# trifectatechfoundation/zlib-rs

Hardware: NVIDIA H100
Metric: deflate_level6_raw_input_throughput_silesia_small_tar (higher is better)
Workload: dtype u8

## Files before the change

__graft_entry__.py:

```python
import os
import subprocess
import sys

ROOT = os.path.dirname(os.path.abspath(__file__))
if ROOT not in sys.path:
    sys.path.insert(0, ROOT)
sys.path.insert(0, os.path.join(ROOT, "tests"))


def build():
    subprocess.check_call(["make", "-C", os.path.join(ROOT, "zlib_rs_b200", "csrc"), "-j8"])
    subprocess.check_call(["make", "-C", os.path.join(ROOT, "oracle")])
    subprocess.check_call(["make", "-C", os.path.join(ROOT, "oracle"), "ref"])
    subprocess.check_call(["make", "-C", os.path.join(ROOT, "tests", "hostmodel")])
    subprocess.check_call(["make", "-C", os.path.join(ROOT, "tests", "shardmodel")])
    subprocess.check_call(["make", "-C", os.path.join(ROOT, "tests", "membermodel")])
    subprocess.check_call(["make", "-C", os.path.join(ROOT, "tests", "bgzfmodel")])
    subprocess.check_call(["make", "-C", os.path.join(ROOT, "tests", "batchmodel")])
    subprocess.check_call(["make", "-C", os.path.join(ROOT, "tests", "batchdictmodel")])
    subprocess.check_call(["make", "-C", os.path.join(ROOT, "tests", "batchdictsmodel")])
    subprocess.check_call(["make", "-C", os.path.join(ROOT, "tests", "batchparammodel")])
    subprocess.check_call(["make", "-C", os.path.join(ROOT, "tests", "indexmodel")])
    subprocess.check_call(["make", "-C", os.path.join(ROOT, "tests", "writerindexmodel")])
    subprocess.check_call(["make", "-C", os.path.join(ROOT, "tests", "flushmodel")])
    subprocess.check_call(["make", "-C", os.path.join(ROOT, "tests", "bgzfindexmodel")])
    subprocess.check_call(["make", "-C", os.path.join(ROOT, "tests", "c_client")])
    import zlib_rs_b200
    zlib_rs_b200.lib()


def smoke():
    import zlib
    import zlib_rs_b200 as Z
    import oracle_lib as O
    from corpus import synthetic_mix
    d = synthetic_mix(300000, seed=1)
    out = Z.compress2(d, 6)
    assert out == O.compress(d, 6)[1], "GPU deflate differs from the oracle"
    assert zlib.decompress(out) == d
    assert Z.uncompress(out, len(d)) == d
    assert Z.crc32(d) == O.crc32(d) and Z.adler32(d) == O.adler32(d)
    print("smoke ok: %d -> %d bytes, bit-exact vs oracle" % (len(d), len(out)))


if __name__ == "__main__":
    build()
    if len(sys.argv) > 1 and sys.argv[1] == "smoke":
        smoke()
```

zlib_rs_b200/csrc/zb_core.h:

```cpp
#pragma once
#include <stdint.h>

#if defined(__CUDACC__)
#define ZB_HD __host__ __device__ __forceinline__
#define ZB_HDN __host__ __device__
#else
#define ZB_HD inline
#define ZB_HDN
#endif

namespace zb {

constexpr uint32_t kWSize = 32768;
constexpr uint32_t kMaxDist = kWSize - 262;
constexpr uint32_t kMinLookahead = 262;
constexpr uint32_t kT0 = 2 * kWSize - 262;
constexpr uint32_t kMaxMatch = 258;
constexpr uint32_t kLitBufsize = 16384;
constexpr uint32_t kBlockSyms = kLitBufsize - 1;
constexpr uint32_t kTailZone = 1024;
constexpr uint32_t kMSafe = 640;
constexpr uint32_t kPad = 1024;

ZB_HD uint32_t zlib_level_flags(uint32_t level, bool plain_strategy)
// ... 19 lines not shown
    }
}
ZB_HD void stream_trailer(uint8_t *t, uint32_t wrap, uint32_t check, uint32_t isize)
{
    if (wrap == 1) {
        for (int i = 0; i < 4; i++) t[i] = (uint8_t)(check >> (24 - 8 * i));
    } else if (wrap == 2) {
        for (int i = 0; i < 4; i++) { t[i] = (uint8_t)(check >> (8 * i)); t[4 + i] = (uint8_t)(isize >> (8 * i)); }
    }
}
constexpr uint32_t kStoredMax = 65535;
ZB_HD uint64_t stored_blocks(uint64_t n) { return n == 0 ? 1 : (n + kStoredMax - 1) / kStoredMax; }
ZB_HD uint64_t stored_payload(uint64_t n) { return n + 5 * stored_blocks(n); }
ZB_HD void stored_header(uint8_t *p, uint32_t len, bool last)
{
    p[0] = last ? 1 : 0;
    p[1] = (uint8_t)len;
    p[2] = (uint8_t)(len >> 8);
    p[3] = (uint8_t)~len;
    p[4] = (uint8_t)(~len >> 8);
}

struct LevelParams {
    uint32_t good, lazy, nice, chain;
    uint32_t early_exit;
};
ZB_HD LevelParams level_params(int level)
{
    switch (level) {
    case 3: return {4, 6, 16, 6, 1};
    case 4: return {4, 12, 32, 24, 1};
    case 5: return {8, 16, 32, 32, 0};
    default: return {8, 16, 128, 128, 0};
    }
}

ZB_HD uint32_t hash_u32(uint32_t v) { return (v * 2654435761u) >> 16; }

struct FullWin {
    ZB_HD uint32_t wsize() const { return kWSize; }
    ZB_HD uint32_t maxdist() const { return kMaxDist; }
    ZB_HD uint32_t t0() const { return kT0; }
};
struct DynWin {
    uint32_t w;
    ZB_HD uint32_t wsize() const { return w; }
    ZB_HD uint32_t maxdist() const { return w - kMinLookahead; }
    ZB_HD uint32_t t0() const { return 2 * w - kMinLookahead; }
};
template <class WN>
ZB_HD uint32_t wbase_w(const WN &wn, uint32_t p) { return p <= wn.t0() ? 0u : wn.wsize() * (1u + (p - wn.t0() - 1u) / wn.wsize()); }

ZB_HD uint32_t wbase(uint32_t p) { return p <= kT0 ? 0u : kWSize * (1u + (p - kT0 - 1u) / kWSize); }


template <class A>
ZB_HD uint32_t common_prefix(const A &a, uint32_t x, uint32_t c, uint32_t maxlen)
{
    uint32_t n = 0;
    while (n < maxlen && a.byte(x + n) == a.byte(c + n)) n++;
    return n;
}

struct Match {
    uint32_t len;
    uint32_t start;
};

template <class A, class WN = FullWin>
ZB_HD Match lm_walk(const A &a, uint32_t x, uint32_t cap, const LevelParams &lp, const WN wn = WN())
{
    Match r{0, 0};
    uint32_t best = 2;
    uint32_t chain = lp.chain;
    uint32_t cur = x;
    bool first = true;
    for (;;) {
        uint32_t d = a.link(cur);
        if (d == 0) break;
        cur -= d;
        uint32_t dist = x - cur;
        if (dist > (first ? wn.maxdist() : wn.maxdist() - 1)) break;
        if (cur == 0) break;
        if (!a.inserted(cur)) continue;
        first = false;
        uint32_t len = 0;
        bool pass;
        if (best < 8) {
            uint32_t c8 = common_prefix(a, x, cur, 8);
            if (c8 == 8) { pass = true; }
            else if (c8 > best) { pass = true; len = c8; }
            else pass = false;
        } else {
            uint32_t off = best - 7;
            pass = common_prefix(a, x + off, cur + off, 8) == 8 && common_prefix(a, x, cur, 8) == 8;
        }
        if (pass) {
            if (len == 0) len = 2 + common_prefix(a, x + 2, cur + 2, 256);
            if (len > best) {
                r.start = cur;
                if (len >= cap) { r.len = cap; return r; }
                best = len;
                r.len = len;
                if (best >= lp.nice) return r;
            } else if (lp.early_exit) {
                break;
// ... 226 lines not shown
```

zlib_rs_b200/csrc/zb_engine.cu:

```cuda
#include <cuda_runtime.h>
#include <stdio.h>
#include <stdlib.h>
#include <string.h>
#include <algorithm>
#include <new>
#include "../../include/zb_engine.h"
#include "zb_kernels.cuh"
#include "zb_engine_internal.h"

namespace zb {

constexpr uint32_t kSlowSub9 = 24576;
constexpr uint32_t kTailTiles = 2;
constexpr uint32_t kTailSub = 512;

thread_local char g_err[256] = "";

static void set_err(const char *what, cudaError_t e)
{
    snprintf(g_err, sizeof g_err, "%s: %s", what, cudaGetErrorString(e));
}

#define CK(call)                                                  \
    do {                                                          \
        cudaError_t e_ = (call);                                  \
        if (e_ != cudaSuccess) { set_err(#call, e_); return ZB_E_CUDA; } \
    } while (0)

__global__ void k_match(JobBufs);
__global__ void k_skip(JobBufs);
__global__ void k_nxt(JobBufs);
__global__ void k_path_tiles(JobBufs);
__global__ void k_path_chain(JobBufs, uint32_t, uint32_t);
__global__ void k_path_groups(JobBufs, uint32_t, uint32_t, uint4 *, uint32_t *);
__global__ void k_path_chain2(JobBufs, uint32_t, uint32_t, const uint4 *, uint32_t *, uint32_t *);
__global__ void k_path_mark(JobBufs, const uint32_t *, const uint32_t *);
__global__ void k_iter_lists(JobBufs, uint32_t *, uint32_t *, uint32_t);
__global__ void k_emit(JobBufs);
__global__ void k_holes(JobBufs, uint32_t);
__global__ void k_holes_cmp(JobBufs, uint32_t, uint32_t);
__global__ void k_tail(JobBufs);
__global__ void k_block_hist(JobBufs, uint32_t *);
__global__ void k_build_blocks(JobBufs, const uint32_t *);
__global__ void k_scan_blocks(JobBufs);
__global__ void k_encode(JobBufs);
__global__ void k_finish(JobBufs, const uint32_t *);
__global__ void k_literal_syms(JobBufs);
__global__ void k_stored(JobBufs);
__global__ void k_links2_std(JobBufs, uint32_t);
__global__ void k_links2_roll(JobBufs, uint32_t);
__global__ void k_links_fix_std(JobBufs);
__global__ void k_links_fix_roll(JobBufs);
__global__ void k_slow(JobBufs);
__global__ void k_rle(JobBufs);
__global__ void k_emit_slow(JobBufs);
__global__ void k_tail_slow(JobBufs);
__global__ void k_serial_low(JobBufs);
__global__ void k_links_dict_ghost(JobBufs, uint32_t *);
__global__ void k_links_dict_ghost_apply(JobBufs, const uint32_t *);
__global__ void k_bgzf_setup(BgzfJob, uint64_t);
__global__ void k_serial_low_members(JobBufs, BgzfJob);
__global__ void k_bgzf_medium(JobBufs, BgzfJob);
__global__ void k_bgzf_slow_steps(JobBufs, BgzfJob);
__global__ void k_bgzf_slow_walk(JobBufs, BgzfJob);
__global__ void k_bgzf_rle_steps(JobBufs, BgzfJob);
__global__ void k_bgzf_literals(JobBufs, BgzfJob);
__global__ void k_bgzf_hist(JobBufs, BgzfJob, uint32_t *);
__global__ void k_bgzf_build(JobBufs, BgzfJob, const uint32_t *);
__global__ void k_bgzf_size(JobBufs, BgzfJob);
__global__ void k_bgzf_scan(JobBufs, BgzfJob);
__global__ void k_bgzf_encode(JobBufs, BgzfJob);
__global__ void k_bgzf_frame(JobBufs, BgzfJob);
__global__ void k_batch_stage(const uint8_t *, const uint64_t *, const uint8_t *, const uint64_t *, BgzfJob, uint8_t *, uint64_t);
__global__ void k_batch_dict_ghost(JobBufs, BgzfJob);
__global__ void k_flush_blocks(JobBufs, BgzfJob);
__global__ void k_deflate_points(JobBufs, BgzfJob, IdxWriteJob);

constexpr uint32_t kMatchSmemBytes = (kWSize + kMatchSub + 512) + (kWSize + kMatchSub) * 2 + ((kWSize + kMatchSub) / 32 + 1) * 4 * 4 + 8192;
constexpr uint32_t kPathSmemBytes = kPathTile * 4 * 3;
constexpr uint32_t kLinks2SmemBytes = 65536 * 2 + kLinkTile * 2 + kLinkTile + 64 + 2048;
constexpr uint32_t kSkipSmemBytes = 2 * kWSize * 2 + 2 * (2 * kWSize / 32) * 4 + 8192 + 64;
constexpr uint32_t kSlowSubMax = 24576;
constexpr uint32_t kSlowSmemBytes = (kWSize + kSlowSubMax + kSlowAhead) * 3;
constexpr uint32_t kChainSmemBytes = kChainChunkTiles * kPathHead * 8;
constexpr uint32_t kChain2MaxSmem = 200 * 1024;
constexpr uint32_t kSerialSmemBytes = (65536 + kWSize) * 2 + 35824 + 16;
constexpr uint32_t kSerialSmemQuick = 65536 * 2 + 65536 + 16;

int Engine::init(int dev)
{
    int n = 0;
    cudaError_t e = cudaGetDeviceCount(&n);
    if (e != cudaSuccess || n == 0) {
        snprintf(g_err, sizeof g_err, "no CUDA device (%s)", e == cudaSuccess ? "count 0" : cudaGetErrorString(e));
        return ZB_E_NODEVICE;
    }
    if (dev < 0 || dev >= n) { snprintf(g_err, sizeof g_err, "device %d out of range", dev); return ZB_E_PARAM; }
    device = dev;
    CK(cudaSetDevice(dev));
    CK(cudaStreamCreateWithFlags(&st, cudaStreamNonBlocking));
    CK(cudaStreamCreateWithFlags(&st2, cudaStreamNonBlocking));
    CK(cudaEventCreateWithFlags(&evf, cudaEventDisableTiming));
    CK(cudaEventCreateWithFlags(&evt, cudaEventDisableTiming));
    for (int i = 0; i < kUpChunks; i++) CK(cudaEventCreateWithFlags(&evc[i], cudaEventDisableTiming));
    CK(cudaEventCreateWithFlags(&evk, cudaEventDisableTiming));
    CK(cudaEventCreate(&ev0));
    CK(cudaEventCreate(&ev1));
    CK(upload_tables());
    CK(cudaFuncSetAttribute(k_match, cudaFuncAttributeMaxDynamicSharedMemorySize, kMatchSmemBytes));
    CK(cudaFuncSetAttribute(k_skip, cudaFuncAttributeMaxDynamicSharedMemorySize, kSkipSmemBytes));
    CK(cudaFuncSetAttribute(k_links2_std, cudaFuncAttributeMaxDynamicSharedMemorySize, kLinks2SmemBytes));
    CK(cudaFuncSetAttribute(k_links2_roll, cudaFuncAttributeMaxDynamicSharedMemorySize, kLinks2SmemBytes));
    CK(cudaFuncSetAttribute(k_slow, cudaFuncAttributeMaxDynamicSharedMemorySize, kSlowSmemBytes));
    CK(cudaFuncSetAttribute(k_path_tiles, cudaFuncAttributeMaxDynamicSharedMemorySize, kPathSmemBytes));
    CK(cudaFuncSetAttribute(k_path_mark, cudaFuncAttributeMaxDynamicSharedMemorySize, kPathSmemBytes));
    CK(cudaFuncSetAttribute(k_path_chain, cudaFuncAttributeMaxDynamicSharedMemorySize, kChainSmemBytes));
    CK(cudaFuncSetAttribute(k_path_groups, cudaFuncAttributeMaxDynamicSharedMemorySize, kChain2MaxSmem));
    CK(cudaFuncSetAttribute(k_path_chain2, cudaFuncAttributeMaxDynamicSharedMemorySize, kChain2MaxSmem));
    CK(cudaFuncSetAttribute(k_serial_low, cudaFuncAttributeMaxDynamicSharedMemorySize, kSerialSmemBytes));
    CK(cudaFuncSetAttribute(k_serial_low_members, cudaFuncAttributeMaxDynamicSharedMemorySize, kSerialSmemBytes));
    CK(cudaMallocHost(&h_info, sizeof(JobInfo)));
    CK(cudaMalloc(&d_info, sizeof(JobInfo)));
    CK(cudaMalloc(&d_check, 16));
    { int rc_ = inflate_init(); if (rc_ != ZB_OK) return rc_; }
    return ZB_OK;
}

Engine::~Engine()
{
    if (device < 0) return;
    cudaSetDevice(device);
    for (auto &b : bufs) if (b.p) cudaFree(b.p);
    if (h_stage) cudaFreeHost(h_stage);
    if (h_info) cudaFreeHost(h_info);
    if (d_info) cudaFree(d_info);
    if (d_check) cudaFree(d_check);
    if (ev0) cudaEventDestroy(ev0);
    if (ev1) cudaEventDestroy(ev1);
    if (evf) cudaEventDestroy(evf);
    if (evt) cudaEventDestroy(evt);
    for (int i = 0; i < kUpChunks; i++) if (evc[i]) cudaEventDestroy(evc[i]);
    if (evk) cudaEventDestroy(evk);
    if (st2) cudaStreamDestroy(st2);
    if (st) cudaStreamDestroy(st);
}

void Engine::pbegin()
{
    if (!profile) return;
    if (!pev0) { cudaEventCreate(&pev0); cudaEventCreate(&pev1); }
    cudaEventRecord(pev0, st);
}

void Engine::pend(int phase, uint32_t nlaunch)
{
    if (!profile) return;
    cudaEventRecord(pev1, st);
    cudaEventSynchronize(pev1);
    float ms = 0;
    cudaEventElapsedTime(&ms, pev0, pev1);
    phase_ms[phase] += ms;
    phase_launches[phase] += nlaunch;
}
// ... 58 lines not shown
    uint32_t wrap;
    if (window_bits < 0) { if (window_bits < -15 || window_bits > -8) return ZB_E_PARAM; wrap = 0; }
    else if (window_bits > 15) { if (window_bits < 24 || window_bits > 31) return ZB_E_PARAM; wrap = 2; }
    else { if (window_bits < 8) return ZB_E_PARAM; wrap = 1; }
    const int wb = window_bits < 0 ? -window_bits : window_bits > 15 ? window_bits - 16 : window_bits;
    CK(cudaSetDevice(device));
    const uint32_t N = (uint32_t)n;
    launches = 0;

    JobBufs jb;
    memset(&jb, 0, sizeof jb);
    int rc;
    void *p;
    const size_t npad = (size_t)N + kPad;
    const uint32_t nwords = (N >> 5) + 2;
    const uint32_t nmt = N / kMatchTile + 1, npt = N / kPathTile + 1;
    const bool low_parallel = (flags & ZB_FLAG_LOW_PARALLEL) != 0 || dstart != 0;
    const bool serial_low = (level == 1 || level == 2) && strategy != 2 && strategy != 3 && !low_parallel;
    const uint32_t block_syms = (serial_low && level == 1) ? kBlockSyms : (1u << (mem_level + 6)) - 1u;
    const uint32_t max_blocks = N / block_syms + 2;
    const size_t out_cap = (deflate_bound(n) + 15) & ~(size_t)15;
    if ((rc = stage((size_t)nmt + 64 + ((size_t)N / 512 + 2 + npt + nmt + 8) * 4 + 64)) != ZB_OK) return rc;
    uint8_t *h_dirty = static_cast<uint8_t *>(h_stage);
    uint32_t *h_lists = reinterpret_cast<uint32_t *>(static_cast<uint8_t *>(h_stage) + (((size_t)nmt + 64 + 15) & ~(size_t)15));
#define RES(slot, bytes, field, type)                                   \
    if ((rc = reserve(slot, bytes, &p)) != ZB_OK) return rc;            \
    jb.field = static_cast<type>(p);
    uint8_t *d_in;
    if ((rc = reserve(S_IN, npad + 16, &p)) != ZB_OK) return rc;
    d_in = static_cast<uint8_t *>(p);
    jb.in = d_in;
    jb.N = N;
    jb.start = (uint32_t)dstart;
    jb.nmt = nmt;
    jb.tail_start = N > 2 * kTailZone ? N - kTailZone : 0;
    jb.block_syms = block_syms;
    jb.serial_mode = serial_low ? (uint32_t)level : 0u;
    RES(S_L, npad * 2, L, uint16_t *)
    RES(S_SK, npad * 2, SK, uint16_t *)
    RES(S_HOLES, (size_t)nwords * 4, holes, uint32_t *)
    RES(S_HOLESN, (size_t)nwords * 4, holes_new, uint32_t *)
    RES(S_M, npad * 4, M, uint32_t *)
    RES(S_NXT, ((size_t)N + 16) * 4, nxt, uint32_t *)
    RES(S_PEXIT, ((size_t)N + 16) * 4, pexit, uint32_t *)
    RES(S_PCNT, ((size_t)N + 16) * 4, pcnt, uint32_t *)
    RES(S_SYMIDX, ((size_t)N + 16) * 4, symidx, uint32_t *)
    RES(S_PHEAD, (size_t)npt * kPathHead * 8, phead, uint2 *)
    RES(S_TENTRY, (size_t)npt * 4, tile_entry, uint32_t *)
    RES(S_TSYMB, (size_t)npt * 4, tile_symbase, uint32_t *)
    RES(S_MARKN, (size_t)npt + 16, mark_needed, uint8_t *)
    const uint32_t nlists = npt * (kPathTile / kPathSub);
    RES(S_LLIST, (size_t)nlists * kLongPerSub * 4, long_list, uint32_t *)
    RES(S_LCNT, (size_t)nlists * 4, long_cnt, uint32_t *)
    RES(S_TDIRTY, (size_t)nmt + 16, tile_dirty, uint8_t *)
    RES(S_SYMS, ((size_t)N + 64) * sizeof(Sym), syms, Sym *)
    RES(S_SYMB, 40000 * 4, sym_base, uint32_t *)
    RES(S_BMAP, (size_t)nmt * 8192, bucket_map, uint32_t *)
    RES(S_LR, npad * 2, Lr, uint16_t *)
    RES(S_KEYS, npad * 2, keys, uint16_t *)
    RES(S_LLAST, (size_t)nmt * 65536 * 2, link_last, uint16_t *)
    RES(S_CSTATE, (size_t)(npt + 1) * 16, chain_state, uint4 *)
    uint32_t chainG = 16;
    while ((uint64_t)chainG * chainG < npt) chainG += 8;
    const uint32_t chain_groups = (npt + chainG - 1) / chainG;
    const uint32_t chain2_smem = chainG * kPathHead * 8 + chain_groups * kPathHead * 16 + chainG * 8;
    const bool chain2 = chain2_smem <= kChain2MaxSmem;
    if ((rc = reserve(S_GFN, (size_t)chain_groups * kPathHead * 16 + ((size_t)npt + 4) * 4, &p)) != ZB_OK) return rc;
    uint4 *d_gfn = static_cast<uint4 *>(p);
    uint32_t *d_mark_cnt = reinterpret_cast<uint32_t *>(d_gfn + (size_t)chain_groups * kPathHead);
    uint32_t *d_mark_list = d_mark_cnt + 4;
    auto launch_chain = [&](uint32_t first_tile) {
        if (chain2) {
            k_path_groups<<<chain_groups, 1024, chainG * kPathHead * 8, st>>>(jb, npt, chainG, d_gfn, d_mark_cnt);
            k_path_chain2<<<chain_groups, 1024, chain2_smem, st>>>(jb, npt, chainG, d_gfn, d_mark_list, d_mark_cnt);
            launches++;
        } else k_path_chain<<<1, 1024, kChainSmemBytes, st>>>(jb, npt, first_tile);
    };
    auto launch_mark = [&](uint32_t grid) {
        if (chain2) k_path_mark<<<grid < npt ? grid : npt, 1024, kPathSmemBytes, st>>>(jb, d_mark_list, d_mark_cnt);
        else k_path_mark<<<npt, 1024, kPathSmemBytes, st>>>(jb, nullptr, nullptr);
    };
    uint32_t *d_lists;
    const uint32_t max_list = N / 512 + 2;
    if ((rc = reserve(S_LISTS, ((size_t)max_list + npt + nmt + 8) * 4, &p)) != ZB_OK) return rc;
    d_lists = static_cast<uint32_t *>(p);
    RES(S_HDIFF, (size_t)nwords * 8, hdiff, uint32_t *)
    jb.hdiff_words = nwords;
    RES(S_HCOARSE, (size_t)(N >> 10) + 16, hcoarse, uint8_t *)
    RES(S_MCHG, (((size_t)N >> 8) + 16) * 4 + 64, mchg, uint8_t *)
    RES(S_BLOCKS, (size_t)max_blocks * sizeof(BlockDesc), blocks, BlockDesc *)
    RES(S_BBASE, (size_t)max_blocks * 4, block_base, uint32_t *)
    uint32_t *d_freq;
    if ((rc = reserve(S_FREQ, (size_t)max_blocks * 320 * 4, &p)) != ZB_OK) return rc;
    d_freq = static_cast<uint32_t *>(p);
    uint8_t *d_out;
    if (dst_dev && dst_cap >= out_cap) d_out = static_cast<uint8_t *>(dst);
    else { if ((rc = reserve(S_OUT, out_cap + 16, &p)) != ZB_OK) return rc; d_out = static_cast<uint8_t *>(p); }
    jb.out = d_out;
    jb.out_cap = out_cap;
    void *d_ck;
    const size_t ck_bytes = ((size_t)N / 16384 + 16) * 8;
    if ((rc = reserve(S_CK, ck_bytes, &d_ck)) != ZB_OK) return rc;
#undef RES
    jb.info = d_info;
    jb.level = (uint32_t)level;
    jb.strategy_fixed = strategy == 4;
    const bool lf_zero = strategy >= 2;
// ... 71 lines not shown
        pend(9, 0);
    }
    CK(cudaMemsetAsync(d_info, 0, sizeof(JobInfo), st));
    CK(cudaMemsetAsync(d_out, 0, out_cap, st));
    if (jb.prime_bits) {
        h_prime = (uint8_t)((flags >> 16) & ((1u << jb.prime_bits) - 1u));
        CK(cudaMemcpyAsync(d_out, &h_prime, 1, cudaMemcpyHostToDevice, st));
    }
    cudaStream_t st_ck = chunked_upload ? st2 : st;
    pbegin();
    if (wrap == 1 || (wrap == 0 && (flags & ZB_FLAG_CHECK_ADLER))) { CK(launch_adler32(d_in + dstart, n_in, 1, d_ck, ck_bytes, d_check, st_ck)); launches += 2; }
    else if (wrap == 2 || (wrap == 0 && (flags & ZB_FLAG_CHECK_CRC))) { CK(launch_crc32(d_in + dstart, n_in, 0, d_ck, ck_bytes, d_check, st_ck)); launches += 2; }
    else CK(cudaMemsetAsync(d_check, 0, 4, st_ck));
    if (chunked_upload) CK(cudaEventRecord(evk, st2));
    pend(8, 2);

    auto links_tiles = [&](bool roll) {
        uint32_t t_done = 0;
        for (uint32_t k = 0; k < (chunked_upload ? up_chunks : 1u); k++) {
            uint32_t t_hi = nmt;
            if (chunked_upload) {
                cudaStreamWaitEvent(st, evc[k], 0);
                if (k + 1 < up_chunks) t_hi = up_len[k] >= 64 ? (uint32_t)((up_len[k] - 64) / kLinkTile) : 0;
            }
            if (t_hi <= t_done) continue;
            if (roll) k_links2_roll<<<t_hi - t_done, 1024, kLinks2SmemBytes, st>>>(jb, t_done);
            else k_links2_std<<<t_hi - t_done, 1024, kLinks2SmemBytes, st>>>(jb, t_done);
            if (k) launches++;
            t_done = t_hi;
        }
        if (chunked_upload) cudaStreamWaitEvent(st, evk, 0);
    };
    uint32_t iters = 0;
    if (level == 0) {
        const uint32_t nb = n_in == 0 ? 1 : (uint32_t)((n_in + 65534) / 65535);
        k_stored<<<nb, 256, 0, st>>>(jb);
        launches++;
        k_finish<<<1, 32, 0, st>>>(jb, d_check);
        launches++;
    } else {
        if (jb.huffman_only) {
            k_literal_syms<<<(uint32_t)(n_in / 256 + 1), 256, 0, st>>>(jb);
            launches++;
        } else if (jb.serial_mode) {
            iters = 1;
            pbegin();
            k_serial_low<<<1, 32, jb.serial_mode == 2 ? kSerialSmemBytes : kSerialSmemQuick, st>>>(jb);
            launches++;
            pend(1, 1);
        } else {
            CK(cudaMemsetAsync(jb.holes, 0, (size_t)nwords * 4, st));
            CK(cudaMemsetAsync(jb.holes_new, 0, (size_t)nwords * 4, st));
            CK(cudaMemsetAsync(jb.tile_dirty, 1, nmt, st));
            CK(cudaMemsetAsync(jb.tile_entry, 0xee, (size_t)npt * 4, st));
            CK(cudaMemsetAsync(jb.M + N, 0, (size_t)kPad * 4, st));
            CK(cudaMemsetAsync(jb.L + N, 0, (size_t)kPad * 2, st));
            pbegin();
            if (jb.slow_mode == 2) {
            } else if (jb.slow_mode && jb.sp.slow) {
                links_tiles(true);
                k_links_fix_roll<<<N / 256 + 1, 256, 0, st>>>(jb);
                launches += 2;
            } else {
                links_tiles(false);
                k_links_fix_std<<<N / 256 + 1, 256, 0, st>>>(jb);
                launches += 2;
                if (dstart >= 3 && n_in) {
                    uint32_t *d_first = reinterpret_cast<uint32_t *>(d_check) + 2;
                    CK(cudaMemsetAsync(d_first, 0xff, 4, st));
                    k_links_dict_ghost<<<(kMaxDist + 255) / 256, 256, 0, st>>>(jb, d_first);
                    k_links_dict_ghost_apply<<<1, 32, 0, st>>>(jb, d_first);
                    launches += 2;
                }
            }
            if (!jb.slow_mode) CK(cudaMemcpyAsync(jb.Lr, jb.L, npad * 2, cudaMemcpyDeviceToDevice, st));
            pend(0, 1);
            if (jb.slow_mode) {
                if (n_in > 0) {
                    iters = 1;
                    pbegin();
                    if (jb.slow_mode == 2) k_rle<<<(N + 255) / 256, 256, 0, st>>>(jb);
                    else {
                        jb.match_sub = level >= 9 ? kSlowSub9 : level == 8 ? 4096u : 8192u;
                        k_slow<<<(N + jb.match_sub - 1) / jb.match_sub, 1024, (kWSize + jb.match_sub + kSlowAhead) * 3, st>>>(jb);
                    }
                    pend(1, 1);
                    if (profile) phase_ms[11] = phase_ms[1];
                    pbegin();
                    k_path_tiles<<<npt, 1024, kPathSmemBytes, st>>>(jb);
                    launch_chain(0);
                    launch_mark(npt);
                    pend(3, 3);
                    pbegin();
                    k_emit_slow<<<(N + 255) / 256, 256, 0, st>>>(jb);
                    pend(4, 1);
                    launches += 5;
                }
                pbegin();
                k_tail_slow<<<1, 32, 0, st>>>(jb);
                launches++;
                pend(5, 1);
            } else {
            if (jb.tail_start > 0) {
                uint32_t n_dirty = nmt;
                for (;;) {
                    iters++;
                    uint32_t mthreads = 1024;
                    if (iters == 1) jb.match_sub = 4096;
                    else if (n_dirty <= kTailTiles) { jb.match_sub = kTailSub; mthreads = 256; }
                    else {
                        const uint64_t per_cta = (uint64_t)n_dirty * kMatchTile / (4 * (uint64_t)device_sm_count());
                        jb.match_sub = per_cta >= 8192 ? 8192 : per_cta >= 4096 ? 4096 : per_cta >= 2048 ? 2048 : 1024;
                    }
                    uint32_t nsub = (N + jb.match_sub - 1) / jb.match_sub;
                    uint32_t n_ptiles = npt, first_ptile = 0;
                    jb.skip_list = nullptr;
                    jb.nxt_list = nullptr;
                    if (iters > 1) {
                        jb.skip_list = d_lists;
                        jb.nxt_list = d_lists + nmt + 8;
                        n_ptiles = h_info->n_ptiles ? h_info->n_ptiles : 1;
                        first_ptile = h_info->first_ptile;
                        nsub = (n_dirty ? n_dirty : 1) * (kMatchTile / jb.match_sub);
                        if (n_dirty) {
                            pbegin();
                            k_skip<<<n_dirty, 1024, kSkipSmemBytes, st>>>(jb);
                            pend(1, 1);
                            launches++;
                        }
                    }
                    const uint32_t msmem = (kWSize + jb.match_sub + 512) + (kWSize + jb.match_sub) * 2 +
                                           (iters > 1 ? ((kWSize + jb.match_sub) / 32 + 1) * 4 * 4 + 8192 : 64);
                    jb.use_bucket_map = iters > 1;
                    pbegin();
                    k_match<<<nsub, mthreads, msmem, st>>>(jb);
                    pend(1, 1);
                    if (profile && iters == 1) phase_ms[11] = phase_ms[1];
                    pbegin();
                    k_nxt<<<n_ptiles * (kPathTile / 1024), 1024, 0, st>>>(jb);
                    pend(2, 1);
                    pbegin();
                    k_path_tiles<<<n_ptiles, 1024, kPathSmemBytes, st>>>(jb);
                    launch_chain(first_ptile);
                    launch_mark(iters == 1 ? npt : 2 * n_ptiles + 16);
                    pend(3, 3);
                    pbegin();
                    k_holes<<<(nlists * kLongPerSub + 255) / 256, 256, 0, st>>>(jb, nlists);
                    k_holes_cmp<<<(nwords + 255) / 256, 256, 0, st>>>(jb, nwords, nmt);
                    pend(4, 2);
                    launches += 7;
                    k_iter_lists<<<1, 1024, 0, st>>>(jb, d_lists, d_lists + nmt + 8, npt);
                    launches++;
                    CK(cudaMemcpyAsync(h_info, d_info, sizeof(JobInfo), cudaMemcpyDeviceToHost, st));
                    CK(cudaStreamSynchronize(st));
                    if (h_info->error) { snprintf(g_err, sizeof g_err, "engine error flags 0x%x (parse)", h_info->error); return ZB_E_INTERNAL; }
                    if (getenv("ZB_DEBUG")) {
                        static unsigned long long last[3];
                        if (iters == 1) memset(last, 0, sizeof last);
                        const double ctas = (double)(h_info->dbg[0] - last[0]) + 1e-9;
                        fprintf(stderr, "iter %u dirty %u: ctas %llu stage %.1f walk %.1f kcyc/cta, holes_changed %u, sub %u first_tile %u chain %u\n",
                                iters, n_dirty, h_info->dbg[0] - last[0], (h_info->dbg[1] - last[1]) / 1e3 / ctas,
                                (h_info->dbg[2] - last[2]) / 1e3 / ctas, h_info->holes_changed, jb.match_sub, first_ptile, chain2 ? 2u : 1u);
                        memcpy(last, h_info->dbg, sizeof last);
                    }
                    if (!h_info->holes_changed) break;
                    n_dirty = h_info->n_dirty;
                    if (iters > N / 257u + 4096u) { snprintf(g_err, sizeof g_err, "hole iteration did not converge"); return ZB_E_INTERNAL; }
                }
            }
            CK(cudaEventRecord(evf, st));
            CK(cudaStreamWaitEvent(st2, evf, 0));
            k_tail<<<1, 32, 0, st2>>>(jb);
            launches++;
            CK(cudaEventRecord(evt, st2));
            if (jb.tail_start > 0) {
                pbegin();
                k_emit<<<(jb.tail_start + 255) / 256, 256, 0, st>>>(jb);
                launches++;
                pend(4, 1);
            }
            pbegin();
// ... 1268 lines not shown
```

zlib_rs_b200/csrc/zb_kernels.cu:

```cuda
#include "zb_kernels.cuh"

namespace zb {

__constant__ HuffTables c_tab;

cudaError_t upload_tables()
{
    HuffTables t;
    init_tables(t);
    return cudaMemcpyToSymbol(c_tab, &t, sizeof t);
}

struct GAcc {
    const uint8_t *data;
    uint32_t N;
    const uint16_t *L;
    const uint32_t *holes;
    const uint32_t *M;
    uint32_t w = kWSize;
    __device__ __forceinline__ uint32_t byte(uint32_t y) const
    {
        while (y >= N) {
            if (y < 2 * w) return 0;
            y -= w;
// ... 109 lines not shown
        const uint32_t lb = c_base[warp], ln = c_total[warp];
        for (uint32_t k = 0; k < ln; k += 32) {
            const bool mine = k + lane < ln;
            const uint32_t m = __ballot_sync(0xffffffffu, mine);
            if (mine) {
                const uint32_t i = lists[lb + k + lane];
                const uint32_t key = key_of(i);
                const uint32_t peers = __match_any_sync(m, key);
                const uint32_t lower = peers & ((1u << lane) - 1u);
                const uint32_t pi = __shfl_sync(m, i, lower ? 31 - __clz(lower) : lane);
                const uint32_t pred = lower ? pi + 1 : head[key];
                uint32_t d = pred ? i + 1 - pred : kFirstFlag;
                if (pred && d > cap) d = 0;
                jb.L[ts + i] = (uint16_t)d;
                if ((peers >> lane) == 1u) head[key] = (uint16_t)(i + 1);
            }
            __syncwarp();
        }
    }
    for (uint32_t x = tv + tid; x < te; x += 1024) jb.L[x] = 0;
    __syncthreads();
    uint4 *out = reinterpret_cast<uint4 *>(jb.link_last + (size_t)tile * kKeys);
    const uint4 *hv = reinterpret_cast<const uint4 *>(head);
    for (uint32_t i = tid; i < kKeys * 2 / 16; i += 1024) out[i] = hv[i];
}

template <bool kRoll>
__device__ __forceinline__ void links_fix_body(const JobBufs &jb)
{
    constexpr uint32_t kKeys = kRoll ? 32768u : 65536u;
    const uint32_t x = blockIdx.x * 256 + threadIdx.x;
    if (x >= jb.N || jb.L[x] != kFirstFlag) return;
    const uint32_t tile = x / kLinkTile, cap = kRoll ? jb.wsize - 1u : jb.wsize - kMinLookahead;
    uint32_t d = 0;
    if (tile > 0) {
        const uint8_t *q = jb.in + x;
        const uint32_t key = kRoll ? hash_roll3(q[0], q[1], q[2])
                                   : hash_u32((uint32_t)q[0] | ((uint32_t)q[1] << 8) | ((uint32_t)q[2] << 16) | ((uint32_t)q[3] << 24));
        const uint32_t last = jb.link_last[(size_t)(tile - 1) * kKeys + key];
        if (last) {
            d = x - ((tile - 1) * kLinkTile + last - 1);
            if (d > cap) d = 0;
        }
    }
    jb.L[x] = (uint16_t)d;
}

__global__ void __launch_bounds__(1024) k_links2_std(JobBufs jb, uint32_t tile0) { links2_body<false>(jb, tile0); }
__global__ void __launch_bounds__(1024) k_links2_roll(JobBufs jb, uint32_t tile0) { links2_body<true>(jb, tile0); }
__global__ void __launch_bounds__(256) k_links_fix_std(JobBufs jb) { links_fix_body<false>(jb); }
__global__ void __launch_bounds__(256) k_links_fix_roll(JobBufs jb) { links_fix_body<true>(jb); }

constexpr uint32_t kSkipSpan = 2 * kWSize;
__global__ void __launch_bounds__(1024) k_skip(JobBufs jb)
{
    extern __shared__ __align__(16) uint8_t smem[];
    uint16_t *sL = reinterpret_cast<uint16_t *>(smem);
    uint32_t *sh = reinterpret_cast<uint32_t *>(smem + kSkipSpan * 2);
    uint32_t *sf = sh + kSkipSpan / 32;
    uint32_t *sbm = sf + kSkipSpan / 32;
    const uint32_t tile = jb.skip_list ? jb.skip_list[blockIdx.x] : blockIdx.x;
    const uint32_t ts = tile * kMatchTile;
    if (ts >= jb.N) return;
    const uint32_t te = min(ts + kMatchTile, jb.N);
    const uint32_t ws = ts >= kWSize ? ts - kWSize : 0;
    const uint32_t span = te - ws, tid = threadIdx.x;
    const uint32_t md = jb.wsize - kMinLookahead;
    {
        const uint4 *ls = reinterpret_cast<const uint4 *>(jb.L + ws);
        uint4 *ld = reinterpret_cast<uint4 *>(sL);
        for (uint32_t i = tid; i < (span + 7) / 8; i += 1024) ld[i] = ls[i];
        for (uint32_t i = tid; i < (span + 31) / 32; i += 1024) sh[i] = jb.holes[(ws >> 5) + i];
        const uint32_t *bm1 = jb.bucket_map + (size_t)tile * 2048, *bm0 = tile ? bm1 - 2048 : bm1;
        for (uint32_t i = tid; i < 2048; i += 1024) sbm[i] = bm0[i] | bm1[i];
    }
    __syncthreads();
    {
        const uint4 *kp = reinterpret_cast<const uint4 *>(jb.keys + ws);
        const uint32_t ngrp = ((span + 31) & ~31u) / 8, ngrp_w = (ngrp + 31) & ~31u;
#pragma unroll 4
        for (uint32_t g = tid; g < ngrp_w; g += 1024) {
            const bool valid = g < ngrp;
            const uint4 kv = valid ? kp[g] : make_uint4(0, 0, 0, 0);
            const uint32_t k[8] = {kv.x & 0xffffu, kv.x >> 16, kv.y & 0xffffu, kv.y >> 16, kv.z & 0xffffu, kv.z >> 16, kv.w & 0xffffu, kv.w >> 16};
            uint32_t b = 0;
#pragma unroll
            for (int j = 0; j < 8; j++) b |= ((sbm[k[j] >> 5] >> (k[j] & 31u)) & 1u) << j;
            b <<= 8 * (tid & 3u);
            b |= __shfl_xor_sync(0xffffffffu, b, 1);
            b |= __shfl_xor_sync(0xffffffffu, b, 2);
            if (valid && (tid & 3u) == 0) sf[g >> 2] = b;
        }
    }
    __syncthreads();
    const uint32_t lane = tid & 31, warp = tid >> 5, nwords = (span + 31) / 32;
    uint32_t nz[2];
#pragma unroll
    for (int h = 0; h < 2; h++) {
        const uint32_t w = warp * 64 + lane + 32 * h;
        nz[h] = __ballot_sync(0xffffffffu, w < nwords && (sh[w] & sf[w]) != 0);
    }
    for (uint32_t round = 0; round < 24; round++) {
        int ch = 0;
#pragma unroll
        for (int h = 0; h < 2; h++) {
            uint32_t m = nz[h];
            while (m) {
                const uint32_t w = warp * 64 + (__ffs(m) - 1) + 32 * h;
                m &= m - 1;
                const uint32_t i = w * 32 + lane;
                const bool on = (((sh[w] & sf[w]) >> lane) & 1u) && i < span;
                for (int rep = 0; rep < 6; rep++) {
                    bool c = false;
                    if (on) {
                        const uint32_t d = sL[i];
                        if (d != 0 && d <= i) {
                            const uint32_t t = i - d;
                            if ((sh[t >> 5] >> (t & 31)) & 1u) {
                                const uint32_t d2 = sL[t];
                                sL[i] = (uint16_t)((d2 == 0 || d + d2 > md) ? 0u : d + d2);
                                c = true;
                            }
                        }
                    }
                    __syncwarp();
                    if (!__any_sync(0xffffffffu, c)) break;
                    ch = 1;
                }
            }
        }
        if (!__syncthreads_or(ch)) break;
    }
    for (uint32_t i = ts - ws + tid; i < span; i += 1024) {
        if (sf[i >> 5] == 0) continue;
        if (!((sf[i >> 5] >> (i & 31)) & 1u)) continue;
        uint32_t d = sL[i];
        if (!((sh[i >> 5] >> (i & 31)) & 1u) && d != 0 && d <= i) {
            const uint32_t t = i - d;
            if ((sh[t >> 5] >> (t & 31)) & 1u) {
                const uint32_t d2 = sL[t];
                d = (d2 == 0 || d + d2 > md) ? 0u : d + d2;
            }
        }
        jb.Lr[ws + i] = (uint16_t)d;
    }
}

constexpr uint32_t kMatchData = kWSize + kMatchSub + 512;
constexpr uint32_t kMatchSmem = kMatchData + (kWSize + kMatchSub) * 2 + ((kWSize + kMatchSub) / 32) * 4;

constexpr uint32_t kBatch = 8;
constexpr uint32_t kBatchCmp = 2;
constexpr uint32_t kWalkBurst = 8;
constexpr uint32_t kCmpBurst = 4;
constexpr uint32_t kCoopCmp = 4;
enum { LS_IDLE = 0, LS_WALK = 1, LS_PEND = 2, LS_DONE = 3, LS_FIN = 4 };

struct DiffMaps {
    const uint32_t *del, *pdel;
    const uint32_t *add, *padd;
    __device__ __forceinline__ static bool any(const uint32_t *b, const uint32_t *p, uint32_t lo, uint32_t hi)
    {
        const uint32_t c_hi = p[hi >> 5] + __popc(b[hi >> 5] & ((1u << (hi & 31)) - 1u));
        const uint32_t c_lo = p[lo >> 5] + __popc(b[lo >> 5] & ((1u << (lo & 31)) - 1u));
        return c_hi != c_lo;
    }
};

__device__ __forceinline__ void sld_u64u(uint32_t a, uint32_t &lo, uint32_t &hi)
{
    const uint32_t al = a & ~3u, sh = (a & 3u) * 8u;
    const uint32_t w0 = sld_u32(al), w1 = sld_u32(al + 4), w2 = sld_u32(al + 8);
    lo = __funnelshift_r(w0, w1, sh);
    hi = __funnelshift_r(w1, w2, sh);
}

__device__ __forceinline__ void match_tile_fast(const JobBufs &jb, const uint8_t *sdata, const uint16_t *sL, const uint32_t *sbm,
                                                const DiffMaps dm, uint32_t ws, uint32_t te, uint32_t *s_next)
{
    const bool filt = jb.use_bucket_map != 0;
    const uint32_t dbase = (uint32_t)__cvta_generic_to_shared(sdata);
    const uint32_t lbase = (uint32_t)__cvta_generic_to_shared(sL);
    const uint32_t N = jb.N, nice = jb.lp.nice, budget = jb.lp.chain;
    const uint32_t md = jb.wsize - kMinLookahead;
    const uint32_t lane = threadIdx.x & 31;
    uint32_t *const Mout = jb.M + ws;
    uint16_t *const RDout = jb.SK + ws;
    uint32_t xr = 0;
    uint32_t cr = 0;
    uint32_t dn = 0;
    uint32_t best = 2, chain = 0, res = 0;
    uint32_t xb = 0;
    uint32_t fbase = 0;
    uint32_t lowr = 0;
    uint32_t clen = 0;
    uint32_t rd = 0;
    uint32_t xw4 = 0;
    uint32_t state = LS_IDLE;
// ... 1541 lines not shown
```

zlib_rs_b200/csrc/zb_kernels.cuh:

```cuda
#pragma once
#include <cuda_runtime.h>
#include "zb_core.h"
#include "zb_huff.h"
#include "zb_slow.h"
#include "zb_bgzf.h"
#include "zb_index.h"

namespace zb {

constexpr uint32_t kLinkTile = 32768;
constexpr uint32_t kMatchTile = 32768;
constexpr uint32_t kMatchSub = 8192;
constexpr uint32_t kPathTile = 16384;
constexpr uint32_t kPathSub = 256;
constexpr uint32_t kLongPerSub = 4;
constexpr uint32_t kPathHead = 64;
constexpr uint32_t kChainChunkTiles = 320;
constexpr uint32_t kNxtTail = 0x80000000u;
constexpr uint32_t kNxtLong = 0x40000000u;
constexpr uint32_t kNxtLong258 = 0x20000000u;
constexpr uint32_t kSymsPerThread = 16;
constexpr uint32_t kSlowAhead = 1024;

__device__ __forceinline__ uint32_t sld_u8(uint32_t a) { uint32_t v; asm volatile("ld.shared.u8 %0, [%1];" : "=r"(v) : "r"(a)); return v; }
__device__ __forceinline__ uint32_t sld_u16(uint32_t a) { uint32_t v; asm volatile("ld.shared.u16 %0, [%1];" : "=r"(v) : "r"(a)); return v; }
__device__ __forceinline__ uint32_t sld_u32(uint32_t a) { uint32_t v; asm volatile("ld.shared.u32 %0, [%1];" : "=r"(v) : "r"(a)); return v; }
__device__ __forceinline__ uint32_t sld_u32u(uint32_t a)
{
    const uint32_t al = a & ~3u;
    return __funnelshift_r(sld_u32(al), sld_u32(al + 4), (a & 3u) * 8u);
}

struct JobInfo {
    uint32_t n_mid_syms;
    uint32_t tail_entry;
    uint32_t n_syms;
    uint32_t final_base;
    uint32_t holes_changed;
    uint32_t n_dirty, n_ptiles, first_ptile;
    uint32_t n_blocks;
    uint32_t data_type;
    uint32_t error;
    uint64_t total_bits;
    uint64_t out_bytes;
    uint32_t adler;
    uint64_t marker_byte;
    unsigned long long dbg[3];
};

struct JobBufs {
    const uint8_t *in;
    uint32_t N;
    uint32_t start;
    uint32_t tail_start;
    uint16_t *L;
    uint16_t *SK;
    uint32_t *hdiff;
    uint32_t hdiff_words;
    uint8_t *hcoarse;
    uint8_t *mchg;
    uint32_t *holes;
    uint32_t *holes_new;
    uint32_t *M;
    uint32_t *nxt;
    uint32_t *pexit;
    uint32_t *pcnt;
    uint2 *phead;
    uint32_t *symidx;
    uint32_t *tile_entry;
    uint32_t *tile_symbase;
    uint8_t *tile_dirty;
    Sym *syms;
    uint32_t *sym_base;
    BlockDesc *blocks;
    TreeScratch *scratch;
    uint8_t *out;
    uint64_t out_cap;
    JobInfo *info;
    LevelParams lp;
    uint32_t level;
    uint32_t strategy_fixed;
    uint32_t wrap;
    uint32_t hdr_len;
    uint32_t xfl;
    uint32_t huffman_only;
    uint32_t match_sub;
    uint32_t nmt;
    uint8_t *mark_needed;
    uint32_t *long_list;
    uint32_t *long_cnt;
    SlowParams sp;
    uint32_t slow_mode;
    uint16_t *link_last;
    uint16_t *Lr;
    uint16_t *keys;
    const uint32_t *skip_list;
    const uint32_t *nxt_list;
    uint4 *chain_state;
    uint32_t *bucket_map;
    uint32_t use_bucket_map;
    uint32_t not_last;
    uint32_t end_mode;
    uint32_t prime_bits;
    uint32_t block_syms;
    uint32_t serial_mode;
    uint32_t *block_base;
    uint32_t wsize;
    uint32_t cinfo;
};

struct BgzfCtl {
    uint32_t count;
    uint32_t error;
    uint32_t n_blocks;
    uint32_t n_syms;
    uint32_t data_type;
    uint32_t pad;
    uint64_t out_bytes;
};
struct BgzfJob {
    uint32_t nm;
    uint32_t wrap;
    uint64_t *moff;
    uint32_t *mlen;
// ... 65 lines not shown
```

Baseline: 1.593.

## Add sliced bounded-hop skip-walk kernel with fallback for few dirty tiles

When only a small number of match tiles are dirty, the skip-link repair is split into 4KB slices per block. Each slice resolves links bridging over holes with a bounded hop walk, which gives more parallelism than one block per tile. Tiles whose walks exceed the hop bound are flagged and reprocessed by the original k_skip kernel in a fallen-only mode. This adds an extra launch and some overhead in exchange for better GPU occupancy in the few-tile case.

```diff
diff --git a/__graft_entry__.py b/__graft_entry__.py
--- a/__graft_entry__.py
+++ b/__graft_entry__.py
@@ -13,6 +13,7 @@
     subprocess.check_call(["make", "-C", os.path.join(ROOT, "oracle")])
     subprocess.check_call(["make", "-C", os.path.join(ROOT, "oracle"), "ref"])
     subprocess.check_call(["make", "-C", os.path.join(ROOT, "tests", "hostmodel")])
+    subprocess.check_call(["make", "-C", os.path.join(ROOT, "tests", "skipmodel")])
     subprocess.check_call(["make", "-C", os.path.join(ROOT, "tests", "shardmodel")])
     subprocess.check_call(["make", "-C", os.path.join(ROOT, "tests", "membermodel")])
     subprocess.check_call(["make", "-C", os.path.join(ROOT, "tests", "bgzfmodel")])
diff --git a/zlib_rs_b200/csrc/zb_core.h b/zlib_rs_b200/csrc/zb_core.h
--- a/zlib_rs_b200/csrc/zb_core.h
+++ b/zlib_rs_b200/csrc/zb_core.h
@@ -95,6 +95,21 @@
 ZB_HD uint32_t wbase_w(const WN &wn, uint32_t p) { return p <= wn.t0() ? 0u : wn.wsize() * (1u + (p - wn.t0() - 1u) / wn.wsize()); }
 
 ZB_HD uint32_t wbase(uint32_t p) { return p <= kT0 ? 0u : kWSize * (1u + (p - kT0 - 1u) / kWSize); }
+
+constexpr uint32_t kBridgeUnbounded = 0xffffffffu;
+ZB_HD uint32_t bridged_link(const uint16_t *L, const uint32_t *holes, uint32_t i, uint32_t md, uint32_t max_hops = 0xffffffffu)
+{
+    uint32_t d = L[i];
+    for (uint32_t hops = 0;; hops++) {
+        if (d == 0 || d > i) return d;
+        const uint32_t t = i - d;
+        if (!((holes[t >> 5] >> (t & 31)) & 1u)) return d;
+        if (hops == max_hops) return kBridgeUnbounded;
+        const uint32_t d2 = L[t];
+        if (d2 == 0 || d + d2 > md) return 0;
+        d += d2;
+    }
+}
 
 
 template <class A>
diff --git a/zlib_rs_b200/csrc/zb_engine.cu b/zlib_rs_b200/csrc/zb_engine.cu
--- a/zlib_rs_b200/csrc/zb_engine.cu
+++ b/zlib_rs_b200/csrc/zb_engine.cu
@@ -28,7 +28,8 @@
     } while (0)
 
 __global__ void k_match(JobBufs);
-__global__ void k_skip(JobBufs);
+__global__ void k_skip(JobBufs, uint32_t);
+__global__ void k_skip_walk(JobBufs);
 __global__ void k_nxt(JobBufs);
 __global__ void k_path_tiles(JobBufs);
 __global__ void k_path_chain(JobBufs, uint32_t, uint32_t);
@@ -80,6 +81,7 @@
 constexpr uint32_t kPathSmemBytes = kPathTile * 4 * 3;
 constexpr uint32_t kLinks2SmemBytes = 65536 * 2 + kLinkTile * 2 + kLinkTile + 64 + 2048;
 constexpr uint32_t kSkipSmemBytes = 2 * kWSize * 2 + 2 * (2 * kWSize / 32) * 4 + 8192 + 64;
+constexpr uint32_t kSkipWalkSmemBytes = (kWSize + kSkipSlice) * 2 + (kWSize + kSkipSlice) / 32 * 4 + 8192;
 constexpr uint32_t kSlowSubMax = 24576;
 constexpr uint32_t kSlowSmemBytes = (kWSize + kSlowSubMax + kSlowAhead) * 3;
 constexpr uint32_t kChainSmemBytes = kChainChunkTiles * kPathHead * 8;
@@ -109,6 +111,7 @@
     CK(upload_tables());
     CK(cudaFuncSetAttribute(k_match, cudaFuncAttributeMaxDynamicSharedMemorySize, kMatchSmemBytes));
     CK(cudaFuncSetAttribute(k_skip, cudaFuncAttributeMaxDynamicSharedMemorySize, kSkipSmemBytes));
+    CK(cudaFuncSetAttribute(k_skip_walk, cudaFuncAttributeMaxDynamicSharedMemorySize, kSkipWalkSmemBytes));
     CK(cudaFuncSetAttribute(k_links2_std, cudaFuncAttributeMaxDynamicSharedMemorySize, kLinks2SmemBytes));
     CK(cudaFuncSetAttribute(k_links2_roll, cudaFuncAttributeMaxDynamicSharedMemorySize, kLinks2SmemBytes));
     CK(cudaFuncSetAttribute(k_slow, cudaFuncAttributeMaxDynamicSharedMemorySize, kSlowSmemBytes));
@@ -273,7 +276,8 @@
     const uint32_t nlists = npt * (kPathTile / kPathSub);
     RES(S_LLIST, (size_t)nlists * kLongPerSub * 4, long_list, uint32_t *)
     RES(S_LCNT, (size_t)nlists * 4, long_cnt, uint32_t *)
-    RES(S_TDIRTY, (size_t)nmt + 16, tile_dirty, uint8_t *)
+    RES(S_TDIRTY, 2 * ((size_t)nmt + 16), tile_dirty, uint8_t *)
+    jb.skip_fall = jb.tile_dirty + nmt + 16;
     RES(S_SYMS, ((size_t)N + 64) * sizeof(Sym), syms, Sym *)
     RES(S_SYMB, 40000 * 4, sym_base, uint32_t *)
     RES(S_BMAP, (size_t)nmt * 8192, bucket_map, uint32_t *)
@@ -451,6 +455,7 @@
             CK(cudaMemsetAsync(jb.holes, 0, (size_t)nwords * 4, st));
             CK(cudaMemsetAsync(jb.holes_new, 0, (size_t)nwords * 4, st));
             CK(cudaMemsetAsync(jb.tile_dirty, 1, nmt, st));
+            CK(cudaMemsetAsync(jb.skip_fall, 0, nmt, st));
             CK(cudaMemsetAsync(jb.tile_entry, 0xee, (size_t)npt * 4, st));
             CK(cudaMemsetAsync(jb.M + N, 0, (size_t)kPad * 4, st));
             CK(cudaMemsetAsync(jb.L + N, 0, (size_t)kPad * 2, st));
@@ -521,11 +526,17 @@
                         n_ptiles = h_info->n_ptiles ? h_info->n_ptiles : 1;
                         first_ptile = h_info->first_ptile;
                         nsub = (n_dirty ? n_dirty : 1) * (kMatchTile / jb.match_sub);
-                        if (n_dirty) {
+                        if (n_dirty > kSkipWalkTiles) {
                             pbegin();
-                            k_skip<<<n_dirty, 1024, kSkipSmemBytes, st>>>(jb);
+                            k_skip<<<n_dirty, 1024, kSkipSmemBytes, st>>>(jb, 0);
                             pend(1, 1);
                             launches++;
+                        } else if (n_dirty) {
+                            pbegin();
+                            k_skip_walk<<<n_dirty * (kMatchTile / kSkipSlice), 1024, kSkipWalkSmemBytes, st>>>(jb);
+                            k_skip<<<n_dirty, 1024, kSkipSmemBytes, st>>>(jb, 1);
+                            pend(1, 2);
+                            launches += 2;
                         }
                     }
                     const uint32_t msmem = (kWSize + jb.match_sub + 512) + (kWSize + jb.match_sub) * 2 +
diff --git a/zlib_rs_b200/csrc/zb_kernels.cu b/zlib_rs_b200/csrc/zb_kernels.cu
--- a/zlib_rs_b200/csrc/zb_kernels.cu
+++ b/zlib_rs_b200/csrc/zb_kernels.cu
@@ -185,7 +185,7 @@
 __global__ void __launch_bounds__(256) k_links_fix_roll(JobBufs jb) { links_fix_body<true>(jb); }
 
 constexpr uint32_t kSkipSpan = 2 * kWSize;
-__global__ void __launch_bounds__(1024) k_skip(JobBufs jb)
+__global__ void __launch_bounds__(1024) k_skip(JobBufs jb, uint32_t fallen_only)
 {
     extern __shared__ __align__(16) uint8_t smem[];
     uint16_t *sL = reinterpret_cast<uint16_t *>(smem);
@@ -195,6 +195,12 @@
     const uint32_t tile = jb.skip_list ? jb.skip_list[blockIdx.x] : blockIdx.x;
     const uint32_t ts = tile * kMatchTile;
     if (ts >= jb.N) return;
+    if (fallen_only) {
+        const bool fell = jb.skip_fall[tile] != 0;
+        __syncthreads();
+        if (!fell) return;
+        if (threadIdx.x == 0) jb.skip_fall[tile] = 0;
+    }
     const uint32_t te = min(ts + kMatchTile, jb.N);
     const uint32_t ws = ts >= kWSize ? ts - kWSize : 0;
     const uint32_t span = te - ws, tid = threadIdx.x;
@@ -277,6 +283,44 @@
         }
         jb.Lr[ws + i] = (uint16_t)d;
     }
+}
+
+__global__ void __launch_bounds__(1024) k_skip_walk(JobBufs jb)
+{
+    extern __shared__ __align__(16) uint8_t smem[];
+    constexpr uint32_t kSpan = kWSize + kSkipSlice;
+    uint16_t *sL = reinterpret_cast<uint16_t *>(smem);
+    uint32_t *sh = reinterpret_cast<uint32_t *>(smem + kSpan * 2);
+    uint32_t *sbm = sh + kSpan / 32;
+    __shared__ uint32_t s_fall;
+    const uint32_t tile = jb.skip_list[blockIdx.x / (kMatchTile / kSkipSlice)];
+    const uint32_t ts = tile * kMatchTile + (blockIdx.x % (kMatchTile / kSkipSlice)) * kSkipSlice;
+    if (ts >= jb.N) return;
+    const uint32_t te = min(ts + kSkipSlice, jb.N);
+    const uint32_t ws = ts >= kWSize ? ts - kWSize : 0;
+    const uint32_t span = te - ws, tid = threadIdx.x;
+    const uint32_t md = jb.wsize - kMinLookahead;
+    {
+        const uint4 *ls = reinterpret_cast<const uint4 *>(jb.L + ws);
+        uint4 *ld = reinterpret_cast<uint4 *>(sL);
+        for (uint32_t i = tid; i < (span + 7) / 8; i += 1024) ld[i] = ls[i];
+        for (uint32_t i = tid; i < (span + 31) / 32; i += 1024) sh[i] = jb.holes[(ws >> 5) + i];
+        const uint32_t *bm1 = jb.bucket_map + (size_t)tile * 2048, *bm0 = tile ? bm1 - 2048 : bm1;
+        for (uint32_t i = tid; i < 2048; i += 1024) sbm[i] = bm0[i] | bm1[i];
+        if (tid == 0) s_fall = 0;
+    }
+    __syncthreads();
+    bool fall = false;
+    for (uint32_t x = ts + tid; x < te; x += 1024) {
+        const uint32_t k = jb.keys[x];
+        if (!((sbm[k >> 5] >> (k & 31u)) & 1u)) continue;
+        const uint32_t v = bridged_link(sL, sh, x - ws, md, kSkipWalkHops);
+        if (v == kBridgeUnbounded) fall = true;
+        else jb.Lr[x] = (uint16_t)v;
+    }
+    if (fall) s_fall = 1;
+    __syncthreads();
+    if (tid == 0 && s_fall) jb.skip_fall[tile] = 1;
 }
 
 constexpr uint32_t kMatchData = kWSize + kMatchSub + 512;
diff --git a/zlib_rs_b200/csrc/zb_kernels.cuh b/zlib_rs_b200/csrc/zb_kernels.cuh
--- a/zlib_rs_b200/csrc/zb_kernels.cuh
+++ b/zlib_rs_b200/csrc/zb_kernels.cuh
@@ -21,6 +21,9 @@
 constexpr uint32_t kNxtLong258 = 0x20000000u;
 constexpr uint32_t kSymsPerThread = 16;
 constexpr uint32_t kSlowAhead = 1024;
+constexpr uint32_t kSkipSlice = 4096;
+constexpr uint32_t kSkipWalkHops = 256;
+constexpr uint32_t kSkipWalkTiles = 32;
 
 __device__ __forceinline__ uint32_t sld_u8(uint32_t a) { uint32_t v; asm volatile("ld.shared.u8 %0, [%1];" : "=r"(v) : "r"(a)); return v; }
 __device__ __forceinline__ uint32_t sld_u16(uint32_t a) { uint32_t v; asm volatile("ld.shared.u16 %0, [%1];" : "=r"(v) : "r"(a)); return v; }
@@ -70,6 +73,7 @@
     uint32_t *tile_entry;
     uint32_t *tile_symbase;
     uint8_t *tile_dirty;
+    uint8_t *skip_fall;
     Sym *syms;
     uint32_t *sym_base;
     BlockDesc *blocks;
```

New measurement: 1.644, median of 6. 1.03x the previous value.
